# sota-zk-labs/zkp-implementation

Hardware: AMD Instinct MI355X
Metric: G1 MSM scalar-muls/sec (higher is better)
Workload: dtype u32 (unsaturated 28-bit-limb Montgomery, 381-bit Fq; 64-bit accumulate)

## Files before the change

### zkp-implementation_amd/csrc/g1_28.hpp

```cpp
#pragma once
#include "fq28.hpp"

namespace zkp {

struct A28 {
    Fq28 x, y;
    static ZKP_DEV A28 load(const uint4* p) {
        A28 a;
        a.x = Fq28::load(p);
        a.y = Fq28::load(p + 4);
        return a;
    }
    ZKP_DEV void store(uint4* p) const {
        x.store(p);
        y.store(p + 4);
    }
};

struct X28 {
    Fq28 x, y, zz, zzz;
    static ZKP_DEV X28 infinity() {
        X28 r;
        r.x = Fq28::zero(); r.y = Fq28::zero(); r.zz = Fq28::zero(); r.zzz = Fq28::zero();
        return r;
    }
    ZKP_DEV bool is_inf() const { return zz.all_zero(); }
    static ZKP_DEV X28 from_affine(const A28& a) {
        X28 r;
        r.x = a.x; r.y = a.y; r.zz = Fq28::one(); r.zzz = Fq28::one();
        return r;
    }
    static ZKP_DEV X28 load(const uint4* p) {
        X28 r;
        r.x = Fq28::load(p); r.y = Fq28::load(p + 4); r.zz = Fq28::load(p + 8); r.zzz = Fq28::load(p + 12);
        return r;
    }
    ZKP_DEV void store(uint4* p) const {
        x.store(p); y.store(p + 4); zz.store(p + 8); zzz.store(p + 12);
    }
    static ZKP_DEV X28 load_s(const uint4* p, uint64_t stride) {
        X28 r;
        r.x = Fq28::load_s(p, stride); r.y = Fq28::load_s(p + 4 * stride, stride);
        r.zz = Fq28::load_s(p + 8 * stride, stride); r.zzz = Fq28::load_s(p + 12 * stride, stride);
        return r;
    }
    ZKP_DEV void store_s(uint4* p, uint64_t stride) const {
        x.store_s(p, stride); y.store_s(p + 4 * stride, stride);
        zz.store_s(p + 8 * stride, stride); zzz.store_s(p + 12 * stride, stride);
    }
};

template <bool CHAIN>
ZKP_DEV Fq28 pmul(const Fq28& a, const Fq28& b) { return CHAIN ? fq28_mul_chain(a, b) : a * b; }
template <bool CHAIN>
ZKP_DEV void pmul2(const Fq28& a0, const Fq28& b0, const Fq28& a1, const Fq28& b1, Fq28& r0, Fq28& r1) {
    if (CHAIN) {
        fq28_mul_chain2(a0, b0, a1, b1, r0, r1);
    } else {
        r0 = a0 * b0;
        r1 = a1 * b1;
    }
}
template <bool CHAIN>
ZKP_DEV Fq28 psqr(const Fq28& a) { return CHAIN ? fq28_sqr_chain(a) : sqr(a); }
template <bool CHAIN = false>
ZKP_DEV void xyzz_finish_neg(Fq28& x3, Fq28& y3, const Fq28& rn, const Fq28& pp, const Fq28& ppp, const Fq28& u1,
                             const Fq28& ns1) {
    Fq28 q = pmul<CHAIN>(u1, pp);
    Fq28 rr = psqr<CHAIN>(rn);
    x3 = normalise(sub8w(sub4(rr, ppp), q + q));
    Fq28 t = sub16(q, x3);
    y3 = CHAIN ? fq28_mul2_chain(rn, t, ns1, ppp) : fq28_mul2(rn, t, ns1, ppp);
}
template <bool CHAIN = false>
ZKP_DEV void xyzz_finish(Fq28& x3, Fq28& y3, const Fq28& r, const Fq28& pp, const Fq28& ppp, const Fq28& u1,
                         const Fq28& s1) {
    xyzz_finish_neg<CHAIN>(x3, y3, normalise(r), pp, ppp, u1, sub8(Fq28::zero(), s1));
}

ZKP_DEV X28 g1_28_double_affine(const A28& p) {
    X28 o;
    Fq28 u = p.y + p.y;
    u = normalise(u);
    Fq28 v = sqr(u);
    Fq28 w = u * v;
    Fq28 s = p.x * v;
    Fq28 xx = sqr(p.x);
    Fq28 m = xx + xx + xx;
    o.x = normalise(sub8w(sqr(m), s + s));
    Fq28 t = sub16(s, o.x);
    o.y = normalise(sub4(m * t, w * p.y));
    o.zz = v;
    o.zzz = w;
    return o;
}

ZKP_DEV X28 g1_28_double(const X28& p) {
    X28 o;
    Fq28 u = p.y + p.y;
    Fq28 v = sqr(u);
    Fq28 w = u * v;
    Fq28 s = p.x * v;
    Fq28 xx = sqr(p.x);
    Fq28 m = xx + xx + xx;
    o.x = normalise(sub8w(sqr(m), s + s));
    Fq28 t = sub16(s, o.x);
    o.y = normalise(sub4(m * t, w * p.y));
    o.zz = v * p.zz;
    o.zzz = w * p.zzz;
    return o;
}

template <bool CHAIN = false>
ZKP_DEV void g1_28_madd(X28& acc, const A28& q) {
    if (acc.is_inf()) {
        acc.x = q.x;
        acc.y = normalise(q.y);
        acc.zz = Fq28::one();
        acc.zzz = Fq28::one();
        return;
    }
    Fq28 u2, s2;
    pmul2<CHAIN>(q.x, acc.zz, q.y, acc.zzz, u2, s2);
    Fq28 p = sub16(u2, acc.x);
    Fq28 ns1 = pinned(neg8(acc.y));
    Fq28 r = s2 + ns1;
    Fq28 pp = psqr<CHAIN>(p);
    if (tight_positive_is_zero_mod_p(pp)) {
        if (tight_is_zero_mod_p(sqr(r))) acc = g1_28_double_affine(q);
        else acc = X28::infinity();
        return;
    }
    Fq28 ppp = pmul<CHAIN>(p, pp);
    Fq28 x3, y3;
    xyzz_finish_neg<CHAIN>(x3, y3, r, pp, ppp, acc.x, ns1);
    acc.x = x3;
    acc.y = y3;
    if (CHAIN) {
        fq28_mul_chain2_inplace(acc.zz, pp, acc.zzz, ppp);
    } else {
        Fq28 zz3, zzz3;
        pmul2<CHAIN>(acc.zz, pp, acc.zzz, ppp, zz3, zzz3);
        acc.zz = zz3;
        acc.zzz = zzz3;
    }
}

template <bool CHAIN = false>
ZKP_DEV bool g1_28_mmadd(X28& acc, const A28& q) {
    Fq28 p = sub16(q.x, acc.x);
    Fq28 pp = psqr<CHAIN>(p);
    if (tight_is_zero_mod_p(pp)) return false;
    Fq28 r = sub8(q.y, acc.y);
    Fq28 ppp = pmul<CHAIN>(p, pp);
    Fq28 x3, y3;
    xyzz_finish<CHAIN>(x3, y3, r, pp, ppp, acc.x, acc.y);
    acc.x = x3;
    acc.y = y3;
    acc.zz = pp;
    acc.zzz = ppp;
    return true;
}

ZKP_DEV void g1_28_add(X28& a, const X28& b) {
    if (b.is_inf()) return;
    if (a.is_inf()) {
        a = b;
        return;
    }
    Fq28 u1 = a.x * b.zz;
    Fq28 u2 = b.x * a.zz;
    Fq28 s1 = a.y * b.zzz;
    Fq28 s2 = b.y * a.zzz;
    Fq28 p = sub4(u2, u1);
    Fq28 r = sub4(s2, s1);
    Fq28 pp = sqr(p);
    if (tight_is_zero_mod_p(pp)) {
        if (tight_is_zero_mod_p(sqr(r))) a = g1_28_double(a);
        else a = X28::infinity();
        return;
    }
    Fq28 ppp = p * pp;
    Fq28 x3, y3;
    xyzz_finish(x3, y3, r, pp, ppp, u1, s1);
    a.x = x3;
    a.y = y3;
    a.zz = a.zz * b.zz * pp;
    a.zzz = a.zzz * b.zzz * ppp;
}

#define ZKP_MEM_FENCE() asm volatile("" ::: "memory")
ZKP_DEV void g1_28_same_x_stream(const uint4* __restrict__ pa, const uint4* __restrict__ pb, uint4* __restrict__ dst, uint64_t st) {
    bool opposite;
    {
        const Fq28 s1 = Fq28::load_s(pa + 4 * st, st) * Fq28::load_s(pb + 12 * st, st);
        const Fq28 s2 = Fq28::load_s(pb + 4 * st, st) * Fq28::load_s(pa + 12 * st, st);
        opposite = !tight_is_zero_mod_p(sqr(sub4(s2, s1)));
    }
    if (opposite) {
        const uint4 z = make_uint4(0u, 0u, 0u, 0u);
#pragma unroll
        for (int q = 0; q < 16; q++) dst[q * st] = z;
        return;
    }
    ZKP_MEM_FENCE();
    Fq28 v, w;
    {
        const Fq28 y = Fq28::load_s(pa + 4 * st, st);
        const Fq28 u = y + y;
        v = sqr(u);
        w = u * v;
    }
    (v * Fq28::load_s(pa + 8 * st, st)).store_s(dst + 8 * st, st);
    (w * Fq28::load_s(pa + 12 * st, st)).store_s(dst + 12 * st, st);
    ZKP_MEM_FENCE();
    Fq28 s, mm;
    {
        const Fq28 x = Fq28::load_s(pa, st);
        s = x * v;
        const Fq28 xx = sqr(x);
        mm = xx + xx + xx;
    }
    const Fq28 x3 = normalise(sub8w(sqr(mm), s + s));
    x3.store_s(dst, st);
    const Fq28 t = sub16(s, x3);
    normalise(sub4(mm * t, w * Fq28::load_s(pa + 4 * st, st))).store_s(dst + 4 * st, st);
}
template <bool CHAIN>
ZKP_DEV void g1_28_add_stream_body(const uint4* pa, const uint4* pb, uint4* dst, uint64_t st) {
    Fq28 u1, p, pp, zz3;
    {
        const Fq28 zz1 = Fq28::load_s(pa + 8 * st, st), zz2 = Fq28::load_s(pb + 8 * st, st);
        const bool inf1 = zz1.all_zero();
        if (inf1 || zz2.all_zero()) {
            const uint4* src = inf1 ? pb : pa;
#pragma unroll
            for (int q = 0; q < 16; q++) dst[q * st] = src[q * st];
            return;
        }
        Fq28 u2;
        pmul2<CHAIN>(Fq28::load_s(pa, st), zz2, Fq28::load_s(pb, st), zz1, u1, u2);
        p = sub4(u2, u1);
        pp = psqr<CHAIN>(p);
        zz3 = pmul<CHAIN>(zz1, zz2);
    }
    if (tight_is_zero_mod_p(pp)) {
        g1_28_same_x_stream(pa, pb, dst, st);
        return;
    }
    pmul<CHAIN>(zz3, pp).store_s(dst + 8 * st, st);
    ZKP_MEM_FENCE();
    const Fq28 ppp = pmul<CHAIN>(p, pp);
    Fq28 s1, r;
    {
        const Fq28 zzz1 = Fq28::load_s(pa + 12 * st, st), zzz2 = Fq28::load_s(pb + 12 * st, st);
        Fq28 s2;
        pmul2<CHAIN>(Fq28::load_s(pa + 4 * st, st), zzz2, Fq28::load_s(pb + 4 * st, st), zzz1, s1, s2);
        r = sub4(s2, s1);
        pmul<CHAIN>(pmul<CHAIN>(zzz1, zzz2), ppp).store_s(dst + 12 * st, st);
    }
    ZKP_MEM_FENCE();
    Fq28 x3, y3;
    xyzz_finish<CHAIN>(x3, y3, r, pp, ppp, u1, s1);
    x3.store_s(dst, st);
    y3.store_s(dst + 4 * st, st);
}
template <bool CHAIN = false>
ZKP_DEV void g1_28_add_stream(const uint4* __restrict__ pa, const uint4* __restrict__ pb, uint4* __restrict__ dst, uint64_t st) {
    g1_28_add_stream_body<CHAIN>(pa, pb, dst, st);
}
template <bool CHAIN = false>
ZKP_DEV void g1_28_add_stream_inplace(uint4* pa, const uint4* __restrict__ pb, uint64_t st) {
    g1_28_add_stream_body<CHAIN>(pa, pb, pa, st);
}

template <int CTRL>
ZKP_DEV Fq28 quad_perm(const Fq28& v) {
    Fq28 r;
#pragma unroll
    for (int i = 0; i < NL28; i++) r.l[i] = (uint32_t)__builtin_amdgcn_mov_dpp((int)v.l[i], CTRL, 0xf, 0xf, true);
    return r;
}
ZKP_DEV Fq28 quad_bcast(const Fq28& v, int src) {
    switch (src & 3) {
        case 0: return quad_perm<0x00>(v);
        case 1: return quad_perm<0x55>(v);
        case 2: return quad_perm<0xaa>(v);
        default: return quad_perm<0xff>(v);
    }
}
ZKP_DEV Fq28 quad_xor1(const Fq28& v) { return quad_perm<0xb1>(v); }
ZKP_DEV int quad_bcast0(int v) { return __builtin_amdgcn_mov_dpp(v, 0x00, 0xf, 0xf, true); }
ZKP_DEV Fq28 fq28_select(bool c, const Fq28& a, const Fq28& b) {
    Fq28 r;
#pragma unroll
    for (int i = 0; i < NL28; i++) r.l[i] = c ? a.l[i] : b.l[i];
    return r;
}
ZKP_DEV void g1_28_add_quad(const uint4* srcA, const uint4* __restrict__ srcB, uint4* dst, uint64_t stride, int j) {
    const bool odd = (j & 1) != 0, hi = (j & 2) != 0;
    const uint4* mine = odd ? srcB : srcA;
    const uint4* other = odd ? srcA : srcB;
    const int zf = hi ? 12 : 8;
    const Fq28 xy = Fq28::load_s(mine + (hi ? 4 : 0) * stride, stride);
    const Fq28 zo = Fq28::load_s(other + zf * stride, stride);
    const Fq28 zm = Fq28::load_s(mine + zf * stride, stride);
    const int inf_mine = zm.all_zero() ? 1 : 0, inf_other = zo.all_zero() ? 1 : 0;
    const int inf_a = quad_bcast0(inf_mine), inf_b = quad_bcast0(inf_other);
    const Fq28 m1 = xy * zo;
    const Fq28 d = sub4(quad_xor1(m1), m1);
    const Fq28 m2 = fq28_select(odd, zo, d) * fq28_select(odd, zm, d);
    const Fq28 pp = quad_bcast(m2, 0);
    const int p_zero = quad_bcast0(tight_is_zero_mod_p(m2) ? 1 : 0);
    if (inf_a | inf_b | p_zero) {
        if (j == 0) {
            X28 a = X28::load_s(srcA, stride);
            const X28 b = X28::load_s(srcB, stride);
            g1_28_add(a, b);
            a.store_s(dst, stride);
        }
        return;
    }
    const Fq28 u1 = quad_bcast(m1, 0);
    const Fq28 m3 = fq28_select(hi, u1, fq28_select(odd, m2, d)) * pp;
    const Fq28 ppp = quad_bcast(m3, 0);
    const Fq28 s1 = quad_bcast(m1, 2);
    const Fq28 x3 = normalise(sub8w(sub4(m2, ppp), m3 + m3));
    const Fq28 t = sub16(m3, x3);
    const Fq28 lhs4 = fq28_select(hi, fq28_select(odd, m2, d), s1);
    const Fq28 rhs4 = fq28_select(hi && !odd, t, ppp);
    const Fq28 m4 = lhs4 * rhs4;
    const Fq28 v = quad_bcast(m4, 0);
    if (j == 2) {
        x3.store_s(dst, stride);
        normalise(sub4(m4, v)).store_s(dst + 4 * stride, stride);
    } else if (j == 1) {
        m3.store_s(dst + 8 * stride, stride);
    } else if (j == 3) {
        m4.store_s(dst + 12 * stride, stride);
    }
}

}
```

### zkp-implementation_amd/csrc/msm.hpp

```cpp
#pragma once
#include "g1.hpp"
#include "g1_28.hpp"
#include "fq28_inv.hpp"
#include "msm_plan.hpp"
#include "glv.hpp"

namespace zkp {

#define ZKP_AT(f, o) offsetof(MsmGeom, f) == o
static_assert(sizeof(MsmGeom) == 160 && ZKP_AT(c, 0) && ZKP_AT(nwin, 4) && ZKP_AT(nb, 8) && ZKP_AT(nchunk, 12) && ZKP_AT(n, 16) && ZKP_AT(chunk, 24) &&
              ZKP_AT(ns, 32) && ZKP_AT(plane_stride, 40) && ZKP_AT(nslice, 48) && ZKP_AT(shared, 52) && ZKP_AT(run_limit, 56) && ZKP_AT(piece, 60) &&
              ZKP_AT(resume, 64) && ZKP_AT(off, 68) && ZKP_AT(interleave, 140) && ZKP_AT(split_log, 144) && ZKP_AT(more, 148) && ZKP_AT(glv, 152), "MsmGeom layout");
#undef ZKP_AT
static_assert(sizeof(SortGeom) == 8 && offsetof(SortGeom, lo_bits) == 0 && offsetof(SortGeom, nhi) == 4, "SortGeom layout");

ZKP_DEV uint64_t bucket_cap(const MsmGeom& g) { return (uint64_t)g.nwin * g.nb; }

#ifdef ZKP_MSM_CHECK
__device__ uint32_t g_msm_check[32];
ZKP_DEV bool msm_check_fail(int cls, uint32_t v0, uint32_t v1) {
    if (atomicAdd(&g_msm_check[cls * 4], 1u) == 0) { g_msm_check[cls * 4 + 1] = v0; g_msm_check[cls * 4 + 2] = v1; }
    return true;
}
#endif
// ... 167 lines not shown
    const uint64_t end = begin + g.chunk < g.n ? begin + g.chunk : g.n;
    const uint32_t* d = digits + (uint64_t)w * g.n;
    uint2* out = entries + (uint64_t)w * g.n;
    const uint32_t lo_mask = (1u << sg.lo_bits) - 1;
    for (uint64_t t0 = begin; t0 < end; t0 += PS_TILE) {
        for (uint32_t k = tid; k < sg.nhi; k += 1024) cnt[k] = 0;
        __syncthreads();
        uint32_t e[PS_PER], rk[PS_PER];
#pragma unroll
        for (int k = 0; k < PS_PER; k++) {
            const uint64_t i = t0 + tid + (uint64_t)k * 1024;
            e[k] = i < end ? d[i] : 0u;
        }
#pragma unroll
        for (int k = 0; k < PS_PER; k++) {
            const uint32_t b = e[k] >> 1;
            rk[k] = b ? atomicAdd(&cnt[(b - 1) >> sg.lo_bits], 1u) : 0u;
        }
        __syncthreads();
        if (tid < 64) wave_exclusive_scan(cnt, base, sg.nhi, tid);
        __syncthreads();
#pragma unroll
        for (int k = 0; k < PS_PER; k++) {
            const uint32_t b = e[k] >> 1;
            if (b) {
                const uint32_t p = (b - 1) >> sg.lo_bits;
                const uint32_t pos = base[p] + rk[k];
                stage[pos] = make_uint2((uint32_t)(t0 - 0 + tid + (uint64_t)k * 1024) | ((e[k] & 1u) << 31), (b - 1) & lo_mask);
                part[pos] = (uint16_t)p;
            }
        }
        __syncthreads();
        const uint32_t total = base[sg.nhi];
        for (uint32_t j = tid; j < total; j += 1024) {
            const uint32_t p = part[j];
#ifdef ZKP_MSM_CHECK
            if ((uint64_t)cur[p] + (j - base[p]) >= g.n && msm_check_fail(0, cur[p] + (j - base[p]), p)) continue;
#endif
            out[cur[p] + (j - base[p])] = stage[j];
        }
        __syncthreads();
        for (uint32_t k = tid; k < sg.nhi; k += 1024) cur[k] += cnt[k];
    }
}

__global__ __launch_bounds__(1024) void msm_binsort_kernel(const uint2* __restrict__ entries, MsmGeom g, SortGeom sg,
                                                           const uint32_t* __restrict__ pstart,
                                                           uint32_t* __restrict__ start, uint32_t* __restrict__ sorted,
                                                           uint32_t* __restrict__ ghist) {
    __shared__ uint32_t h[SORT_MAX_BINS + 1], cnt[SORT_MAX_BINS], base[SORT_MAX_BINS + 1];
    __shared__ uint32_t szh[256];
    __shared__ uint32_t stage[BS_TILE];
    __shared__ uint16_t bin[BS_TILE];
    const uint32_t hi = blockIdx.x, w = blockIdx.y, tid = threadIdx.x;
    const uint32_t lo_n = 1u << sg.lo_bits;
    const uint32_t* ps = pstart + (uint64_t)w * (sg.nhi + 1);
    const uint32_t begin = ps[hi], end = ps[hi + 1];
    const uint2* in = entries + (uint64_t)w * g.n;
    if (tid < lo_n) cnt[tid] = 0;
    if (tid < 256) szh[tid] = 0;
    __syncthreads();
    const uint32_t nt = blockDim.x;
    for (uint32_t i = begin + tid; i < end; i += 4 * nt) {
        uint32_t y[4];
#pragma unroll
        for (int k = 0; k < 4; k++) y[k] = i + k * nt < end ? in[i + k * nt].y : 0xffffffffu;
#pragma unroll
        for (int k = 0; k < 4; k++)
            if (y[k] != 0xffffffffu) atomicAdd(&cnt[y[k]], 1u);
    }
    __syncthreads();
    if (tid < lo_n) atomicAdd(&szh[255 - (cnt[tid] < 255 ? cnt[tid] : 255)], 1u);
    if (tid < 64) wave_exclusive_scan(cnt, h, lo_n, tid);
    __syncthreads();
    if (tid < 256 && szh[tid]) atomicAdd(&ghist[w * 256 + tid], szh[tid]);
    if (tid < lo_n) h[tid] += begin;
    __syncthreads();
    uint32_t* sw = start + (uint64_t)w * (g.nb + 2);
    if (tid < lo_n) sw[(hi << sg.lo_bits) + tid + 1] = h[tid];
    if (hi == 0 && tid == 0) sw[0] = 0;
    if (hi == sg.nhi - 1 && tid == 0) sw[g.nb + 1] = end;
    __syncthreads();
    uint32_t* out = sorted + (uint64_t)w * g.n;
    for (uint32_t t0 = begin; t0 < end; t0 += BS_TILE) {
        if (tid < lo_n) cnt[tid] = 0;
        __syncthreads();
        uint2 e[BS_PER];
        uint32_t rk[BS_PER];
#pragma unroll
        for (int k = 0; k < BS_PER; k++) {
            const uint32_t i = t0 + tid + k * 1024;
            e[k] = i < end ? in[i] : make_uint2(0u, 0xffffffffu);
        }
#pragma unroll
        for (int k = 0; k < BS_PER; k++) rk[k] = e[k].y != 0xffffffffu ? atomicAdd(&cnt[e[k].y], 1u) : 0u;
        __syncthreads();
        if (tid < 64) wave_exclusive_scan(cnt, base, lo_n, tid);
        __syncthreads();
#pragma unroll
        for (int k = 0; k < BS_PER; k++)
            if (e[k].y != 0xffffffffu) {
                const uint32_t pos = base[e[k].y] + rk[k];
                stage[pos] = e[k].x;
                bin[pos] = (uint16_t)e[k].y;
            }
        __syncthreads();
        const uint32_t total = base[lo_n];
        for (uint32_t j = tid; j < total; j += 1024) {
            const uint32_t p = bin[j];
#ifdef ZKP_MSM_CHECK
            if ((uint64_t)h[p] + (j - base[p]) >= g.n && msm_check_fail(1, h[p] + (j - base[p]), p)) continue;
#endif
            out[h[p] + (j - base[p])] = stage[j];
        }
        __syncthreads();
        if (tid < lo_n) h[tid] += cnt[tid];
    }
}


__global__ __launch_bounds__(1024) void msm_rank_kernel(const uint32_t* __restrict__ start, MsmGeom g,
                                                        const uint32_t* __restrict__ ghist, uint32_t* __restrict__ gcur,
                                                        uint32_t* __restrict__ perm) {
    __shared__ uint32_t hist[256], base[256], gh[256], first[257];
    const uint32_t w = blockIdx.y, tid = threadIdx.x;
    const uint32_t* sw = start + (uint64_t)w * (g.nb + 2);
    if (tid < 256) {
        hist[tid] = 0;
        gh[tid] = ghist[w * 256 + tid];
    }
    __syncthreads();
    if (tid < 64) wave_exclusive_scan(gh, first, 256, tid);
    const uint32_t b = 1 + blockIdx.x * 1024 + tid;
    uint32_t bin = 0, rk = 0;
    if (b <= g.nb) {
        const uint32_t sz = sw[b + 1] - sw[b];
        bin = 255 - (sz < 255 ? sz : 255);
        rk = atomicAdd(&hist[bin], 1u);
    }
    __syncthreads();
    if (tid < 256 && hist[tid]) base[tid] = first[tid] + atomicAdd(&gcur[w * 256 + tid], hist[tid]);
    __syncthreads();
#ifdef ZKP_MSM_CHECK
    if (b <= g.nb && base[bin] + rk >= g.nb && msm_check_fail(5, base[bin] + rk, b)) return;
#endif
    if (b <= g.nb) perm[(uint64_t)w * g.nb + base[bin] + rk] = b;
}

__global__ __launch_bounds__(1024) void msm_order_kernel(const uint32_t* __restrict__ start, MsmGeom g,
                                                         const uint32_t* __restrict__ ghist,
                                                         const uint32_t* __restrict__ perm, uint32_t* __restrict__ over,
                                                         uint32_t* __restrict__ over_b, uint32_t* __restrict__ over_off,
                                                         uint4* __restrict__ desc, uint32_t over_cap, uint32_t desc_cap) {
    __shared__ uint32_t s_over[2], gh[256], first[257];
    const uint32_t w = blockIdx.x, tid = threadIdx.x, nt = blockDim.x;
    const uint32_t* sw = start + (uint64_t)w * (g.nb + 2);
    const uint32_t* pw = perm + (uint64_t)w * g.nb;
    if (tid < 256) gh[tid] = ghist[w * 256 + tid];
    __syncthreads();
    if (tid < 64) wave_exclusive_scan(gh, first, 256, tid);
    __syncthreads();
    if (tid == 0) {
        const uint32_t limit_bin = g.run_limit < 254 ? g.run_limit : 254;
        s_over[0] = first[255 - limit_bin];
    }
    __syncthreads();
    const uint32_t n_over = s_over[0] < over_cap ? s_over[0] : over_cap;
#ifdef ZKP_MSM_CHECK
    if (tid == 0 && s_over[0] > g.nb) msm_check_fail(7, s_over[0], over_cap);
#endif
    uint32_t* ob = over_b + (uint64_t)w * over_cap;
    uint32_t* oo = over_off + (uint64_t)w * (over_cap + 1);
    {
        __shared__ uint32_t part[1024];
        const uint32_t per = (n_over + nt - 1) / nt;
        const uint32_t r0 = tid * per < n_over ? tid * per : n_over;
        const uint32_t r1 = r0 + per < n_over ? r0 + per : n_over;
        uint32_t local = 0;
        for (uint32_t r = r0; r < r1; r++) {
            const uint32_t b = pw[r];
#ifdef ZKP_MSM_CHECK
            if ((b == 0 || b > g.nb) && msm_check_fail(6, b, r)) continue;
#endif
            const uint32_t sz = sw[b + 1] - sw[b];
            local += sz > g.run_limit ? (sz + g.piece - 1) / g.piece : 0;
        }
        part[tid] = local;
        __syncthreads();
        for (uint32_t off = 1; off < nt; off <<= 1) {
            const uint32_t v = tid >= off ? part[tid - off] : 0;
            __syncthreads();
            part[tid] += v;
            __syncthreads();
        }
        uint32_t run = tid ? part[tid - 1] : 0;
        for (uint32_t r = r0; r < r1; r++) {
            const uint32_t b = pw[r];
#ifdef ZKP_MSM_CHECK
            if (b == 0 || b > g.nb) { ob[r] = 1; oo[r] = run; continue; }
#endif
            const uint32_t sz = sw[b + 1] - sw[b];
            ob[r] = b;
            oo[r] = run;
            run += sz > g.run_limit ? (sz + g.piece - 1) / g.piece : 0;
        }
        if (tid == nt - 1) {
            const uint32_t total = part[nt - 1];
            oo[n_over] = total;
            s_over[1] = total;
            over[2 * w] = n_over;
            over[2 * w + 1] = total < desc_cap ? total : desc_cap;
        }
    }
    __syncthreads();
    const uint32_t n_pieces = s_over[1] < desc_cap ? s_over[1] : desc_cap;
    uint4* dw = desc + (uint64_t)w * desc_cap;
    for (uint32_t j = tid; j < n_pieces; j += nt) {
        uint32_t lo = 0, hi = n_over;
        while (hi - lo > 1) {
            const uint32_t mid = (lo + hi) >> 1;
            if (oo[mid] <= j) lo = mid; else hi = mid;
        }
        const uint32_t b = ob[lo], p = j - oo[lo];
        const uint32_t first = sw[b] + p * g.piece;
        const uint32_t last = first + g.piece < sw[b + 1] ? first + g.piece : sw[b + 1];
        dw[j] = make_uint4(b, p, first, last);
    }
}

__global__ __launch_bounds__(MSM_THREADS) void g1_to_internal_kernel(const uint4* __restrict__ in, uint64_t n,
                                                                    uint4* __restrict__ out) {
    const uint64_t i = (uint64_t)blockIdx.x * MSM_THREADS + threadIdx.x;
    if (i >= n) return;
    G1Affine p = G1Affine::load(in + i * 6);
#pragma unroll 1
    for (int k = 0; k < 8; k++) {
        p.x = dbl(p.x);
        p.y = dbl(p.y);
    }
    A28 q;
    q.x = fq28_from_sat(p.x);
    q.y = fq28_from_sat(p.y);
    q.store(out + i * 8);
}

struct SliceOffsets {
    uint16_t off[36];
};
__global__ __launch_bounds__(MSM_THREADS) void g1_expand_planes_kernel(uint4* __restrict__ planes, uint4* __restrict__ scratch,
                                                                      uint64_t off, uint64_t cnt, uint64_t plane_stride,
                                                                      uint32_t nplanes, SliceOffsets so) {
    const uint64_t j = (uint64_t)blockIdx.x * MSM_THREADS + threadIdx.x;
    if (j >= cnt) return;
    const uint64_t i = off + j;
    auto slot = [&](uint32_t s, uint32_t t) { return scratch + (((uint64_t)s * 3 + t) * cnt + j) * 4; };
    const A28 p0 = A28::load(planes + i * 8);
    X28 x = g1_28_double_affine(p0);
    Fq28 run = Fq28::one();
#pragma unroll 1
    for (uint32_t s = 1; s < nplanes; s++) {
#pragma unroll 1
        for (uint32_t k = (s == 1 ? 1u : 0u), c = (uint32_t)so.off[s] - so.off[s - 1]; k < c; k++) x = g1_28_double(x);
        A28 raw;
        raw.x = x.x;
        raw.y = x.y;
        raw.store(planes + (s * plane_stride + i) * 8);
        run.store(slot(s, 2));
        x.zz.store(slot(s, 0));
        x.zzz.store(slot(s, 1));
        run = run * x.zzz;
    }
    Fq28 inv = fq28_inverse_gcd(run);
#pragma unroll 1
    for (uint32_t s = nplanes - 1; s >= 1; s--) {
        const Fq28 zi3 = inv * Fq28::load(slot(s, 2));
        inv = inv * Fq28::load(slot(s, 1));
        const Fq28 zi = zi3 * Fq28::load(slot(s, 0));
        const Fq28 zi2 = zi * zi;
        uint4* dst = planes + (s * plane_stride + i) * 8;
        const A28 raw = A28::load(dst);
        A28 q;
        q.x = raw.x * zi2;
        q.y = raw.y * zi3;
        q.store(dst);
    }
}

ZKP_DEV uint4* split_dst(const MsmGeom& g, uint4* buckets, uint4* parts, uint32_t part) {
    return part ? parts + (uint64_t)(part - 1) * 16 * bucket_cap(g) : buckets;
}
ZKP_DEV void split_run(const MsmGeom& g, uint32_t part, uint32_t& lo, uint32_t& hi) {
    if (!g.split_log) return;
    const uint32_t len = hi - lo;
    hi = lo + (uint32_t)(((uint64_t)len * (part + 1)) >> g.split_log);
    lo = lo + (uint32_t)(((uint64_t)len * part) >> g.split_log);
}


#ifdef ZKP_ACC_PLAIN_PRODUCTS
constexpr bool ACC_CHAIN = false;
#else
constexpr bool ACC_CHAIN = true;
#endif
ZKP_DEV void msm_accumulate_run(const uint4* __restrict__ bases28, const uint32_t* __restrict__ idx, uint32_t lo,
                                uint32_t hi, const MsmGeom& g, uint4* dst, uint64_t dst_stride, bool resume,
                                const uint4* src = nullptr, uint64_t src_stride = 1) {
#ifdef ZKP_MSM_CHECK
    if ((lo > hi || hi > g.n) && msm_check_fail(3, lo, hi)) return;
#endif
    if (resume && lo == hi) {
        if (src != dst) X28::load_s(src, src_stride).store_s(dst, dst_stride);
        return;
    }
    X28 acc = resume ? X28::load_s(src, src_stride) : X28::infinity();
    const PlaneDiv pd = plane_div_make(g.shared ? (uint32_t)g.ns : 1u);
    const uint64_t plane_gap = g.plane_stride - g.ns;
    auto locate = [&](uint32_t e) {
        uint64_t pt = e & 0x7fffffffu;
#ifdef ZKP_MSM_CHECK
        if (pt >= g.n && msm_check_fail(2, e, (uint32_t)g.n)) pt = 0;
#endif
        if (g.shared) pt += (uint64_t)plane_div(pd, (uint32_t)pt) * plane_gap;
        return bases28 + pt * 8;
    };
    uint32_t k = lo;
    if (!resume && hi - lo >= 2) {
        const uint32_t e0 = idx[k], e1 = idx[k + 1];
        {
            A28 p0 = A28::load(locate(e0));
            if (e0 >> 31) p0.y = neg4(p0.y);
            acc.x = p0.x;
            acc.y = normalise(p0.y);
        }
        A28 p1 = A28::load(locate(e1));
        if (e1 >> 31) p1.y = normalise(neg4(p1.y));
        if (g1_28_mmadd<ACC_CHAIN>(acc, p1)) {
            k += 2;
        } else {
            acc.zz = Fq28::one();
            acc.zzz = Fq28::one();
            k += 1;
        }
    }
    for (; k < hi; k++) {
        const uint32_t e = idx[k];
        A28 p = A28::load(locate(e));
        if (e >> 31) p.y = neg4(p.y);
        g1_28_madd<ACC_CHAIN>(acc, p);
    }
    acc.store_s(dst, dst_stride);
}

ZKP_DEV void msm_accumulate_body(const uint4* __restrict__ bases28, const uint32_t* __restrict__ sorted,
                                 const uint32_t* __restrict__ start, const uint32_t* __restrict__ perm,
                                 const uint32_t* __restrict__ over, const uint4* __restrict__ desc, uint32_t desc_cap,
                                 uint32_t bucket_blocks, uint32_t extra_blocks, const MsmGeom& g, uint4* __restrict__ buckets,
                                 uint4* __restrict__ pieces, uint4* __restrict__ parts, uint4* __restrict__ carry) {
    const uint32_t per_set = bucket_blocks + extra_blocks;
    const uint32_t w = g.interleave ? blockIdx.x % g.nwin : blockIdx.x / per_set;
    const uint32_t slot = g.interleave ? blockIdx.x / g.nwin : blockIdx.x % per_set;
    const uint32_t* sw = start + (uint64_t)w * (g.nb + 2);
    const uint32_t* idx = sorted + (uint64_t)w * g.n;
    if (slot < bucket_blocks) {
        const uint32_t unit = slot * ACC_THREADS + threadIdx.x;
        const uint32_t rank = unit >> g.split_log, part = unit & ((1u << g.split_log) - 1);
        if (rank >= g.nb) return;
        const uint32_t b = perm[(uint64_t)w * g.nb + rank];
#ifdef ZKP_MSM_CHECK
        if ((b == 0 || b > g.nb) && msm_check_fail(3, b, rank | 0x80000000u)) return;
#endif
        uint32_t lo = sw[b], hi = sw[b + 1];
        const uint64_t e = (uint64_t)w * g.nb + pyr_pos(b - 1, g.nb);
        uint4* dst = g.more ? carry + e * 16 : split_dst(g, buckets, parts, part) + e;
        if (hi - lo > g.run_limit && rank < over[2 * w]) {
            if (part) hi = lo;
            else return;
        }
        split_run(g, part, lo, hi);
        msm_accumulate_run(bases28, idx, lo, hi, g, dst, g.more ? 1 : bucket_cap(g), g.resume != 0, carry + e * 16, 1);
    } else {
        const uint32_t n_pieces = over[2 * w + 1];
#ifdef ZKP_MSM_CHECK
        if (n_pieces > desc_cap && msm_check_fail(4, n_pieces, desc_cap)) return;
#endif
        const uint32_t stride = extra_blocks * ACC_THREADS;
        for (uint32_t j = (slot - bucket_blocks) * ACC_THREADS + threadIdx.x; j < n_pieces; j += stride) {
            const uint4 d = desc[(uint64_t)w * desc_cap + j];
            msm_accumulate_run(bases28, idx, d.z, d.w, g, pieces + ((uint64_t)w * desc_cap + j) * 16, 1, false);
        }
    }
}

__global__ __launch_bounds__(ACC_THREADS) __attribute__((amdgpu_waves_per_eu(3))) void msm_accumulate_kernel(const uint4* __restrict__ bases28,
                                                                    const uint32_t* __restrict__ sorted,
                                                                    const uint32_t* __restrict__ start,
                                                                    const uint32_t* __restrict__ perm,
                                                                    const uint32_t* __restrict__ over,
                                                                    const uint4* __restrict__ desc, uint32_t desc_cap,
                                                                    uint32_t bucket_blocks, uint32_t extra_blocks, MsmGeom g,
                                                                    uint4* __restrict__ buckets,
                                                                    uint4* __restrict__ pieces, uint4* __restrict__ parts,
                                                                    uint4* __restrict__ carry, ClkRec* __restrict__ clk) {
    uint64_t t0 = 0, r0 = 0;
    clk_begin(clk, t0, r0);
    msm_accumulate_body(bases28, sorted, start, perm, over, desc, desc_cap, bucket_blocks, extra_blocks, g, buckets, pieces, parts, carry);
    clk_end(clk, t0, r0);
}

constexpr int MAD_PROBE_ITERS = 8192, MAD_PROBE_CHAINS = 8;
__global__ __launch_bounds__(256) void mad_rate_probe_kernel(uint32_t* __restrict__ out, uint32_t seed, ClkRec* __restrict__ clk) {
    uint64_t t0 = 0, r0 = 0;
    clk_begin(clk, t0, r0);
    const uint32_t a = seed + threadIdx.x, b = seed * 3 + blockIdx.x;
    uint64_t acc[MAD_PROBE_CHAINS];
    uint32_t lo[MAD_PROBE_CHAINS];
#pragma unroll
    for (int c = 0; c < MAD_PROBE_CHAINS; c++) { acc[c] = a + c; lo[c] = b + c; }
#pragma unroll 1
    for (int it = 0; it < MAD_PROBE_ITERS; it++) {
#pragma unroll
        for (int c = 0; c < MAD_PROBE_CHAINS; c++)
            asm volatile("v_mad_u64_u32 %0, vcc, %1, %2, %0" : "+v"(acc[c]) : "v"(a), "v"(lo[c]) : "vcc");
    }
    uint32_t r = 0;
#pragma unroll
    for (int c = 0; c < MAD_PROBE_CHAINS; c++) r ^= (uint32_t)acc[c] ^ (uint32_t)(acc[c] >> 32);
    out[blockIdx.x * blockDim.x + threadIdx.x] = r;
    clk_end(clk, t0, r0);
}

ZKP_DEV void msm_accumulate_quad_run(const uint4* __restrict__ bases28, const uint32_t* __restrict__ idx, uint32_t lo,
                                     uint32_t hi, const MsmGeom& g, uint4* __restrict__ dst, uint64_t dst_stride, int j) {
    const bool odd = (j & 1) != 0, up = (j & 2) != 0;
    Fq28 own = Fq28::zero();
    bool inf = true, fresh = false;
    auto point_of = [&](uint32_t e) -> const uint4* {
        uint64_t pt = e & 0x7fffffffu;
        if (g.shared) {
            const uint32_t ns32 = (uint32_t)g.ns, s = (uint32_t)pt / ns32;
            pt = (uint64_t)s * g.plane_stride + ((uint32_t)pt - s * ns32);
        }
        return bases28 + pt * 8;
    };
    uint32_t e_next = lo < hi ? idx[lo] : 0u, e_next2 = lo + 1 < hi ? idx[lo + 1] : 0u;
    Fq28 c_next = Fq28::zero();
    if (lo < hi) c_next = Fq28::load(point_of(e_next) + (up ? 4 : 0));
    for (uint32_t k = lo; k < hi; k++) {
        const uint32_t e = e_next;
        const uint4* src = point_of(e);
        Fq28 coord = c_next;
        if (k + 1 < hi) {
            e_next = e_next2;
            c_next = Fq28::load(point_of(e_next) + (up ? 4 : 0));
        }
        if (k + 2 < hi) e_next2 = idx[k + 2];
        if (up && (e >> 31)) coord = neg4(coord);
        if (inf) {
            own = odd ? Fq28::one() : (up ? normalise(coord) : coord);
            inf = false;
            fresh = true;
            continue;
        }
        Fq28 m1;
        if (fresh) m1 = normalise(coord);
        else m1 = coord * own;
        fresh = false;
        const Fq28 d = sub16(quad_xor1(m1), own);
        const Fq28 m2 = d * d;
        const Fq28 pp = quad_bcast(m2, 0);
        if (quad_bcast0(tight_is_zero_mod_p(m2) ? 1 : 0)) {
            X28 acc;
            acc.x = quad_bcast(own, 0); acc.zz = quad_bcast(own, 1); acc.y = quad_bcast(own, 2); acc.zzz = quad_bcast(own, 3);
            A28 q = A28::load(src);
            if (e >> 31) q.y = neg4(q.y);
            g1_28_madd(acc, q);
            inf = acc.is_inf();
            own = up ? (odd ? acc.zzz : acc.y) : (odd ? acc.zz : acc.x);
            continue;
        }
        const Fq28 x1 = quad_bcast(own, 0);
        const Fq28 m3 = fq28_select(j == 0, d, fq28_select(j == 3, x1, own)) * pp;
        const Fq28 ppp = quad_bcast(m3, 0), q = quad_bcast(m3, 3);
        const Fq28 x3 = normalise(sub8w(sub4(m2, ppp), q + q));
        const Fq28 t = sub16(q, x3);
        const Fq28 y1 = quad_bcast(own, 2);
        const Fq28 m4 = fq28_select(j == 0, y1, fq28_select(j == 2, d, own)) * fq28_select(j == 2, t, ppp);
        const Fq28 v = quad_bcast(m4, 0);
        const Fq28 x3b = quad_bcast(x3, 2);
        own = up ? (odd ? m4 : normalise(sub4(m4, v))) : (odd ? m3 : x3b);
    }
    uint4* part = dst + (up ? (odd ? 12 : 4) : (odd ? 8 : 0)) * dst_stride;
    if (inf) own = Fq28::zero();
    own.store_s(part, dst_stride);
}

ZKP_DEV void msm_accumulate_quad_body(const uint4* __restrict__ bases28, const uint32_t* __restrict__ sorted,
                                      const uint32_t* __restrict__ start, const uint32_t* __restrict__ perm,
                                      const uint32_t* __restrict__ over, const uint4* __restrict__ desc, uint32_t desc_cap,
                                      uint32_t bucket_blocks, uint32_t extra_blocks, const MsmGeom& g, uint4* __restrict__ buckets,
                                      uint4* __restrict__ pieces, uint4* __restrict__ parts) {
    constexpr uint32_t QUADS = ACC_THREADS / 4;
    const uint32_t per_set = bucket_blocks + extra_blocks;
    const uint32_t w = g.interleave ? blockIdx.x % g.nwin : blockIdx.x / per_set;
    const uint32_t slot = g.interleave ? blockIdx.x / g.nwin : blockIdx.x % per_set;
    const uint32_t* sw = start + (uint64_t)w * (g.nb + 2);
    const uint32_t* idx = sorted + (uint64_t)w * g.n;
    const int j = threadIdx.x & 3;
    const uint32_t quad = threadIdx.x >> 2;
    if (slot < bucket_blocks) {
        const uint32_t unit = slot * QUADS + quad;
        const uint32_t rank = unit >> g.split_log, part = unit & ((1u << g.split_log) - 1);
        if (rank >= g.nb) return;
        const uint32_t b = perm[(uint64_t)w * g.nb + rank];
        uint32_t lo = sw[b], hi = sw[b + 1];
        uint4* dst = split_dst(g, buckets, parts, part) + ((uint64_t)w * g.nb + pyr_pos(b - 1, g.nb));
        if (hi - lo > g.run_limit && rank < over[2 * w]) {
            if (part) hi = lo;
            else return;
        }
        split_run(g, part, lo, hi);
        msm_accumulate_quad_run(bases28, idx, lo, hi, g, dst, bucket_cap(g), j);
    } else {
        const uint32_t n_pieces = over[2 * w + 1];
        const uint32_t stride = extra_blocks * QUADS;
        for (uint32_t p = (slot - bucket_blocks) * QUADS + quad; p < n_pieces; p += stride) {
            const uint4 d = desc[(uint64_t)w * desc_cap + p];
            msm_accumulate_quad_run(bases28, idx, d.z, d.w, g, pieces + ((uint64_t)w * desc_cap + p) * 16, 1, j);
        }
    }
}
__global__ __launch_bounds__(ACC_THREADS) void msm_accumulate_quad_kernel(const uint4* __restrict__ bases28,
                                                                         const uint32_t* __restrict__ sorted,
                                                                         const uint32_t* __restrict__ start,
                                                                         const uint32_t* __restrict__ perm,
                                                                         const uint32_t* __restrict__ over,
                                                                         const uint4* __restrict__ desc, uint32_t desc_cap,
                                                                         uint32_t bucket_blocks, uint32_t extra_blocks, MsmGeom g,
                                                                         uint4* __restrict__ buckets,
                                                                         uint4* __restrict__ pieces, uint4* __restrict__ parts,
                                                                         ClkRec* __restrict__ clk) {
    uint64_t t0 = 0, r0 = 0;
    clk_begin(clk, t0, r0);
    msm_accumulate_quad_body(bases28, sorted, start, perm, over, desc, desc_cap, bucket_blocks, extra_blocks, g, buckets, pieces, parts);
    clk_end(clk, t0, r0);
}

__global__ __launch_bounds__(MSM_THREADS) void msm_fold_parts_kernel(uint4* __restrict__ buckets, uint4* __restrict__ parts,
                                                                    uint64_t cap, uint32_t step) {
    const uint64_t e = (uint64_t)blockIdx.x * (MSM_THREADS / 4) + (threadIdx.x >> 2);
    if (e >= cap) return;
    const uint32_t ia = blockIdx.y << (step + 1), ib = ia + (1u << step);
    uint4* pa = (ia ? parts + (uint64_t)(ia - 1) * 16 * cap : buckets) + e;
    const uint4* pb = parts + (uint64_t)(ib - 1) * 16 * cap + e;
    g1_28_add_quad(pa, pb, pa, cap, threadIdx.x & 3);
}

__global__ __launch_bounds__(MSM_THREADS) void msm_fold_parts_lane_kernel(uint4* __restrict__ buckets, uint4* __restrict__ parts,
                                                                         uint64_t cap, uint32_t step) {
    const uint64_t e = (uint64_t)blockIdx.x * MSM_THREADS + threadIdx.x;
    if (e >= cap) return;
    const uint32_t ia = blockIdx.y << (step + 1), ib = ia + (1u << step);
    uint4* pa = (ia ? parts + (uint64_t)(ia - 1) * 16 * cap : buckets) + e;
    const uint4* pb = parts + (uint64_t)(ib - 1) * 16 * cap + e;
    g1_28_add_stream_inplace<ACC_CHAIN>(pa, pb, cap);
}

__global__ __launch_bounds__(64) void msm_combine_kernel(const uint32_t* __restrict__ over, const uint32_t* __restrict__ over_b,
                                                         const uint32_t* __restrict__ over_off, uint32_t over_cap,
                                                         uint32_t desc_cap, MsmGeom g, const uint4* __restrict__ pieces,
                                                         uint4* __restrict__ buckets, uint4* __restrict__ carry) {
    __shared__ uint4 sh[64 * 16];
    const uint32_t w = blockIdx.y, lane = threadIdx.x;
    for (uint32_t r = blockIdx.x; r < over[2 * w]; r += gridDim.x) {
    const uint32_t b = over_b[(uint64_t)w * over_cap + r];
    const uint32_t* oo = over_off + (uint64_t)w * (over_cap + 1);
    uint32_t p0 = oo[r], p1 = oo[r + 1];
    if (p1 > desc_cap) p1 = desc_cap;
    if (p1 <= p0) continue;
    const uint4* pw = pieces + (uint64_t)w * desc_cap * 16;
    X28 acc = X28::infinity();
    for (uint32_t p = p0 + lane; p < p1; p += 64) {
        X28 x = X28::load(pw + (uint64_t)p * 16);
        g1_28_add(acc, x);
    }
    for (uint32_t off = 32; off > 0; off >>= 1) {
        acc.store(sh + lane * 16);
        __syncthreads();
        if (lane < off) {
            X28 x = X28::load(sh + (lane + off) * 16);
            g1_28_add(acc, x);
        }
        __syncthreads();
    }
    if (lane == 0) {
        const uint64_t e = (uint64_t)w * g.nb + pyr_pos(b - 1, g.nb);
        if (g.resume) {
            X28 x = X28::load_s(carry + e * 16, 1);
            g1_28_add(acc, x);
        }
        if (g.more) acc.store_s(carry + e * 16, 1);
        else acc.store_s(buckets + e, bucket_cap(g));
    }
    __syncthreads();
    }
}


__global__ __launch_bounds__(MSM_THREADS) void msm_pyramid_kernel(const uint4* __restrict__ pyr_in,
                                                                  uint4* pyr_out,
                                                                  const uint4* __restrict__ odd_in,
                                                                  uint4* __restrict__ odd_out, PyrLevel L) {
    const uint32_t s = blockIdx.x * MSM_THREADS + threadIdx.x;
    if (s >= L.half) return;
    const uint32_t kind = blockIdx.y, w = blockIdx.z;
    const uint64_t cap = (uint64_t)L.nwin * L.nb;
    const PyrItem it = pyr_item(L.nb, L.level, L.half, kind, s, (uint64_t)w * L.nb);
    const uint4* src = kind == 0 ? pyr_in : (it.src_is_pyr_out ? pyr_out : odd_in);
    g1_28_add_stream<ACC_CHAIN>(src + it.a, src + it.b, (kind ? odd_out : pyr_out) + it.d, cap);
}

__global__ __launch_bounds__(MSM_THREADS) void msm_pyramid_quad_kernel(const uint4* __restrict__ pyr_in,
                                                                       uint4* pyr_out,
                                                                       const uint4* __restrict__ odd_in,
                                                                       uint4* __restrict__ odd_out, PyrLevel L) {
    const uint32_t s = blockIdx.x * (MSM_THREADS / 4) + (threadIdx.x >> 2);
    const int j = threadIdx.x & 3;
    if (s >= L.half) return;
    const uint32_t kind = blockIdx.y, w = blockIdx.z;
    const uint64_t cap = (uint64_t)L.nwin * L.nb;
    const PyrItem it = pyr_item(L.nb, L.level, L.half, kind, s, (uint64_t)w * L.nb);
    const uint4* src = kind == 0 ? pyr_in : (it.src_is_pyr_out ? pyr_out : odd_in);
    g1_28_add_quad(src + it.a, src + it.b, (kind ? odd_out : pyr_out) + it.d, cap, j);
}

constexpr uint32_t MSM_TAIL_TIMEOUT = 0x80000000u;
constexpr uint32_t MSM_FLAG_PENDING = 0x40000000u;
constexpr uint32_t MSM_FLAG_PENDING_MASK = 0x40000000u;
constexpr uint32_t PYR_TAIL_SPIN_LIMIT = 1u << 24;
__global__ __launch_bounds__(512) void msm_pyramid_tail_kernel(uint4* __restrict__ pyr0, uint4* __restrict__ pyr1,
                                                               uint4* __restrict__ odd0, uint4* __restrict__ odd1,
                                                               uint32_t level0, uint32_t c, uint32_t nb,
                                                               uint32_t* __restrict__ barrier ,
                                                               uint4* __restrict__ result ,
                                                               uint32_t* __restrict__ flags ,
                                                               uint32_t expect_blocks ,
                                                               uint32_t spin_limit) {
    const uint32_t w = blockIdx.y;
    const uint64_t wbase = (uint64_t)w * nb;
    const uint64_t cap = (uint64_t)gridDim.y * nb;
    const int j = threadIdx.x & 3;
    const uint32_t quad = blockIdx.x * (blockDim.x >> 2) + (threadIdx.x >> 2), nquad = gridDim.x * (blockDim.x >> 2);
    uint32_t epoch = 0;
    for (uint32_t l = level0; l + 1 < c; l++) {
        const uint32_t half = nb >> (l + 1);
        const uint4* pyr_in = (l & 1) ? pyr1 : pyr0;
        uint4* pyr_out = (l & 1) ? pyr0 : pyr1;
        const uint4* odd_in = (l & 1) ? odd1 : odd0;
        uint4* odd_out = (l & 1) ? odd0 : odd1;
        for (uint32_t item = quad; item < (l + 1) * half; item += nquad) {
            const uint32_t kind = item / half, s = item % half;
            const PyrItem it = pyr_item(nb, l, half, kind, s, wbase);
            const uint4* src = kind == 0 ? pyr_in : (it.src_is_pyr_out ? pyr_out : odd_in);
            g1_28_add_quad(src + it.a, src + it.b, (kind ? odd_out : pyr_out) + it.d, cap, j);
        }
        epoch++;
        __syncthreads();
        if (threadIdx.x == 0) {
            uint32_t* bar = barrier + (uint64_t)w * PYR_BAR_STRIDE;
            __builtin_amdgcn_fence(__ATOMIC_RELEASE, "agent");
            __hip_atomic_fetch_add(bar, 1u, __ATOMIC_RELAXED, __HIP_MEMORY_SCOPE_AGENT);
            bool arrived = false;
            for (uint32_t spin = 0; spin < spin_limit; spin++) {
                if (__hip_atomic_load(bar, __ATOMIC_RELAXED, __HIP_MEMORY_SCOPE_AGENT) >= epoch * expect_blocks) {
                    arrived = true;
                    break;
                }
                __builtin_amdgcn_s_sleep(1);
            }
            if (!arrived) __hip_atomic_fetch_or(bar, MSM_TAIL_TIMEOUT, __ATOMIC_RELAXED, __HIP_MEMORY_SCOPE_AGENT);
            __builtin_amdgcn_fence(__ATOMIC_ACQUIRE, "agent");
        }
        __syncthreads();
    }
    if (blockIdx.x == 0) {
        const uint4* pyr_final = ((c - 1) & 1) ? pyr1 : pyr0;
        const uint4* pyr_prev = ((c - 1) & 1) ? pyr0 : pyr1;
        const uint4* odd_final = ((c - 1) & 1) ? odd1 : odd0;
        for (uint32_t t = threadIdx.x; t < c * 16; t += blockDim.x) {
            const uint32_t e = t >> 4, q = t & 15;
            const uint4* src = pyr_result(pyr_final, pyr_prev, odd_final, wbase, nb, c, e);
            result[((uint64_t)w * c + e) * 16 + q] = src[q * cap];
        }
// ... 79 lines not shown
```

Baseline: 441.6 million.

## Run branch-free blind accumulation with careful fallback on degenerate bucket results

Bucket accumulation now runs a blind variant of the mixed and affine-affine additions that skips the infinity and doubling checks. Each run ends with a single test on zz: if it collapsed to zero, the bucket is recomputed with the original careful path. This removes per-add divergent branches and zero-mod-p checks from the hot loop. The cost is extra code size and register pressure, plus occasional recomputation when an exceptional case occurs. Piece runs always use the careful path.

```diff
diff --git a/zkp-implementation_amd/csrc/g1_28.hpp b/zkp-implementation_amd/csrc/g1_28.hpp
--- a/zkp-implementation_amd/csrc/g1_28.hpp
+++ b/zkp-implementation_amd/csrc/g1_28.hpp
@@ -111,9 +111,9 @@
     return o;
 }
 
-template <bool CHAIN = false>
+template <bool CHAIN = false, bool BLIND = false>
 ZKP_DEV void g1_28_madd(X28& acc, const A28& q) {
-    if (acc.is_inf()) {
+    if (!BLIND && acc.is_inf()) {
         acc.x = q.x;
         acc.y = normalise(q.y);
         acc.zz = Fq28::one();
@@ -126,7 +126,7 @@
     Fq28 ns1 = pinned(neg8(acc.y));
     Fq28 r = s2 + ns1;
     Fq28 pp = psqr<CHAIN>(p);
-    if (tight_positive_is_zero_mod_p(pp)) {
+    if (!BLIND && tight_positive_is_zero_mod_p(pp)) {
         if (tight_is_zero_mod_p(sqr(r))) acc = g1_28_double_affine(q);
         else acc = X28::infinity();
         return;
@@ -146,11 +146,11 @@
     }
 }
 
-template <bool CHAIN = false>
+template <bool CHAIN = false, bool BLIND = false>
 ZKP_DEV bool g1_28_mmadd(X28& acc, const A28& q) {
     Fq28 p = sub16(q.x, acc.x);
     Fq28 pp = psqr<CHAIN>(p);
-    if (tight_is_zero_mod_p(pp)) return false;
+    if (!BLIND && tight_is_zero_mod_p(pp)) return false;
     Fq28 r = sub8(q.y, acc.y);
     Fq28 ppp = pmul<CHAIN>(p, pp);
     Fq28 x3, y3;
diff --git a/zkp-implementation_amd/csrc/msm.hpp b/zkp-implementation_amd/csrc/msm.hpp
--- a/zkp-implementation_amd/csrc/msm.hpp
+++ b/zkp-implementation_amd/csrc/msm.hpp
@@ -493,27 +493,33 @@
 #else
 constexpr bool ACC_CHAIN = true;
 #endif
-ZKP_DEV void msm_accumulate_run(const uint4* __restrict__ bases28, const uint32_t* __restrict__ idx, uint32_t lo,
-                                uint32_t hi, const MsmGeom& g, uint4* dst, uint64_t dst_stride, bool resume,
-                                const uint4* src = nullptr, uint64_t src_stride = 1) {
-#ifdef ZKP_MSM_CHECK
-    if ((lo > hi || hi > g.n) && msm_check_fail(3, lo, hi)) return;
-#endif
-    if (resume && lo == hi) {
-        if (src != dst) X28::load_s(src, src_stride).store_s(dst, dst_stride);
-        return;
-    }
+struct AccLocate {
+    const uint4* bases28;
+    PlaneDiv pd;
+    uint64_t plane_gap;
+    bool shared;
+#ifdef ZKP_MSM_CHECK
+    uint64_t n;
+#endif
+    ZKP_DEV AccLocate(const uint4* bases, const MsmGeom& g)
+        : bases28(bases), pd(plane_div_make(g.shared ? (uint32_t)g.ns : 1u)), plane_gap(g.plane_stride - g.ns), shared(g.shared != 0) {
+#ifdef ZKP_MSM_CHECK
+        n = g.n;
+#endif
+    }
+    ZKP_DEV const uint4* operator()(uint32_t e) const {
+        uint64_t pt = e & 0x7fffffffu;
+#ifdef ZKP_MSM_CHECK
+        if (pt >= n && msm_check_fail(2, e, (uint32_t)n)) pt = 0;
+#endif
+        if (shared) pt += (uint64_t)plane_div(pd, (uint32_t)pt) * plane_gap;
+        return bases28 + pt * 8;
+    }
+};
+
+ZKP_DEV X28 msm_accumulate_run_careful(const AccLocate& locate, const uint32_t* __restrict__ idx, uint32_t lo, uint32_t hi, bool resume,
+                                       const uint4* src, uint64_t src_stride) {
     X28 acc = resume ? X28::load_s(src, src_stride) : X28::infinity();
-    const PlaneDiv pd = plane_div_make(g.shared ? (uint32_t)g.ns : 1u);
-    const uint64_t plane_gap = g.plane_stride - g.ns;
-    auto locate = [&](uint32_t e) {
-        uint64_t pt = e & 0x7fffffffu;
-#ifdef ZKP_MSM_CHECK
-        if (pt >= g.n && msm_check_fail(2, e, (uint32_t)g.n)) pt = 0;
-#endif
-        if (g.shared) pt += (uint64_t)plane_div(pd, (uint32_t)pt) * plane_gap;
-        return bases28 + pt * 8;
-    };
     uint32_t k = lo;
     if (!resume && hi - lo >= 2) {
         const uint32_t e0 = idx[k], e1 = idx[k + 1];
@@ -539,7 +545,48 @@
         if (e >> 31) p.y = neg4(p.y);
         g1_28_madd<ACC_CHAIN>(acc, p);
     }
-    acc.store_s(dst, dst_stride);
+    return acc;
+}
+
+ZKP_DEV bool msm_accumulate_run(const AccLocate& locate, const uint32_t* __restrict__ idx, uint32_t lo, uint32_t hi, bool resume,
+                                const uint4* src, uint64_t src_stride, X28& acc) {
+    uint32_t k = lo;
+    bool finite = false;
+    if (!resume && hi - lo >= 2) {
+        const uint32_t e0 = idx[k], e1 = idx[k + 1];
+        {
+            A28 p0 = A28::load(locate(e0));
+            if (e0 >> 31) p0.y = neg4(p0.y);
+            acc.x = p0.x;
+            acc.y = normalise(p0.y);
+        }
+        A28 p1 = A28::load(locate(e1));
+        if (e1 >> 31) p1.y = normalise(neg4(p1.y));
+        g1_28_mmadd<ACC_CHAIN, true>(acc, p1);
+        k += 2;
+        finite = true;
+    } else {
+        acc = resume ? X28::load_s(src, src_stride) : X28::infinity();
+        finite = !acc.is_inf();
+        if (!finite && k < hi) {
+            const uint32_t e = idx[k];
+            A28 p = A28::load(locate(e));
+            if (e >> 31) p.y = neg4(p.y);
+            acc.x = p.x;
+            acc.y = normalise(p.y);
+            acc.zz = Fq28::one();
+            acc.zzz = Fq28::one();
+            k += 1;
+            finite = true;
+        }
+    }
+    for (; k < hi; k++) {
+        const uint32_t e = idx[k];
+        A28 p = A28::load(locate(e));
+        if (e >> 31) p.y = neg4(p.y);
+        g1_28_madd<ACC_CHAIN, true>(acc, p);
+    }
+    return finite && tight_is_zero_mod_p(acc.zz);
 }
 
 ZKP_DEV void msm_accumulate_body(const uint4* __restrict__ bases28, const uint32_t* __restrict__ sorted,
@@ -552,7 +599,15 @@
     const uint32_t slot = g.interleave ? blockIdx.x / g.nwin : blockIdx.x % per_set;
     const uint32_t* sw = start + (uint64_t)w * (g.nb + 2);
     const uint32_t* idx = sorted + (uint64_t)w * g.n;
-    if (slot < bucket_blocks) {
+    const AccLocate locate(bases28, g);
+    const bool bucket_slot = slot < bucket_blocks;
+    const bool resume = bucket_slot && g.resume != 0;
+    uint32_t lo = 0, hi = 0, j = 0, n_pieces = 0;
+    uint4* dst = nullptr;
+    uint64_t dst_stride = 1;
+    const uint4* src = nullptr;
+    bool todo;
+    if (bucket_slot) {
         const uint32_t unit = slot * ACC_THREADS + threadIdx.x;
         const uint32_t rank = unit >> g.split_log, part = unit & ((1u << g.split_log) - 1);
         if (rank >= g.nb) return;
@@ -560,25 +615,48 @@
 #ifdef ZKP_MSM_CHECK
         if ((b == 0 || b > g.nb) && msm_check_fail(3, b, rank | 0x80000000u)) return;
 #endif
-        uint32_t lo = sw[b], hi = sw[b + 1];
+        lo = sw[b];
+        hi = sw[b + 1];
         const uint64_t e = (uint64_t)w * g.nb + pyr_pos(b - 1, g.nb);
-        uint4* dst = g.more ? carry + e * 16 : split_dst(g, buckets, parts, part) + e;
+        dst = g.more ? carry + e * 16 : split_dst(g, buckets, parts, part) + e;
+        dst_stride = g.more ? 1 : bucket_cap(g);
+        src = carry + e * 16;
         if (hi - lo > g.run_limit && rank < over[2 * w]) {
             if (part) hi = lo;
             else return;
         }
         split_run(g, part, lo, hi);
-        msm_accumulate_run(bases28, idx, lo, hi, g, dst, g.more ? 1 : bucket_cap(g), g.resume != 0, carry + e * 16, 1);
+#ifdef ZKP_MSM_CHECK
+        if ((lo > hi || hi > g.n) && msm_check_fail(3, lo, hi)) return;
+#endif
+        if (resume && lo == hi) {
+            if (src != dst) X28::load_s(src, 1).store_s(dst, dst_stride);
+            return;
+        }
+        X28 acc;
+        todo = msm_accumulate_run(locate, idx, lo, hi, resume, src, 1, acc);
+        if (!todo) acc.store_s(dst, dst_stride);
     } else {
-        const uint32_t n_pieces = over[2 * w + 1];
+        n_pieces = over[2 * w + 1];
 #ifdef ZKP_MSM_CHECK
         if (n_pieces > desc_cap && msm_check_fail(4, n_pieces, desc_cap)) return;
 #endif
-        const uint32_t stride = extra_blocks * ACC_THREADS;
-        for (uint32_t j = (slot - bucket_blocks) * ACC_THREADS + threadIdx.x; j < n_pieces; j += stride) {
+        j = (slot - bucket_blocks) * ACC_THREADS + threadIdx.x;
+        todo = j < n_pieces;
+    }
+    while (todo) {
+        if (!bucket_slot) {
             const uint4 d = desc[(uint64_t)w * desc_cap + j];
-            msm_accumulate_run(bases28, idx, d.z, d.w, g, pieces + ((uint64_t)w * desc_cap + j) * 16, 1, false);
-        }
+            lo = d.z;
+            hi = d.w;
+            dst = pieces + ((uint64_t)w * desc_cap + j) * 16;
+#ifdef ZKP_MSM_CHECK
+            if ((lo > hi || hi > g.n) && msm_check_fail(3, lo, hi)) return;
+#endif
+        }
+        msm_accumulate_run_careful(locate, idx, lo, hi, resume, src, 1).store_s(dst, dst_stride);
+        j += extra_blocks * ACC_THREADS;
+        todo = !bucket_slot && j < n_pieces;
     }
 }
 
```

New measurement: 430.1 million. -2.6%, worse.
